# UCSC-nanopore-cgl/margin

Hardware: AMD Instinct MI355X
Metric: het-sites x reads phased/sec (30x ONT synthetic chunks, end to end: every merge level + final sweep) (higher is better)
Workload: dtype int32

## Files before the change

margin_amd/csrc/mrp_kernels.hip:

```cpp
#include <hip/hip_runtime.h>
#include <stdint.h>

#include "mrp_device.h"
#include "mrp_internal.h"
#include "mrp_kernels.h"
#include "mrp_wave.h"
#include "../../include/margin_rphmm.h"

static __device__ __forceinline__ double i32_to_log(int32_t v) {
    return v == MRP_NEG_I32 ? -__builtin_inf() : (double) v;
}
static __device__ __forceinline__ int32_t add_i32(int32_t a, int32_t b) {
    return a == MRP_NEG_I32 ? MRP_NEG_I32 : a + b;
}

__global__ void __launch_bounds__(256) mrp_planes_kernel(const PlaneCol *__restrict__ pcols_all,
                                                         const int32_t *__restrict__ list, int64_t n_cols,
                                                         const int64_t *__restrict__ read_byte_off,
                                                         uint64_t *__restrict__ planes,
                                                         uint32_t *__restrict__ slot_total,
                                                         uint32_t *__restrict__ slot_bytes, int filter) {
    const int lane = threadIdx.x & (WAVE - 1);
    const int wave = __builtin_amdgcn_readfirstlane((int) (threadIdx.x / WAVE));
    const int64_t wave_stride = (int64_t) gridDim.x * (blockDim.x / WAVE);
    int64_t col = (int64_t) blockIdx.x * (blockDim.x / WAVE) + wave;
    if (col >= n_cols) return;
#define PLANE_COL(i) (pcols_all + (list ? (int64_t) __builtin_amdgcn_readfirstlane(list[i]) : (i)))
    PlaneCol c = k_load(PLANE_COL(col));
    int64_t my_off = lane < c.depth ? read_byte_off[c.read_off + lane] : 0;
    for (; col < n_cols; col += wave_stride) {
    const int64_t ncol = col + wave_stride < n_cols ? col + wave_stride : col;
    const PlaneCol cn = k_load(PLANE_COL(ncol));
    const int64_t next_off = lane < cn.depth ? read_byte_off[cn.read_off + lane] : 0;
    const bool active = lane < c.depth;
    const uint8_t *__restrict__ src = c.pool + my_off;
#define PLANE_U 8
    const int n_slots_here = (filter && !c.need_planes) ? 0 : c.n_slots;
    for (int s0 = 0; s0 < n_slots_here; s0 += PLANE_U) {
        uint32_t bytes[PLANE_U];
#pragma unroll
        for (int u = 0; u < PLANE_U; u++) bytes[u] = (active && s0 + u < c.n_slots) ? src[s0 + u] : 0u;
#pragma unroll
        for (int u = 0; u < PLANE_U; u++) {
            const int s = s0 + u;
            if (s < c.n_slots) {
                const uint32_t byte = bytes[u];
                uint32_t packed = byte << (8 * (lane & 3));
                packed |= __shfl_xor(packed, 1, WAVE);
                packed |= __shfl_xor(packed, 2, WAVE);
                if ((lane & 3) == 0) slot_bytes[(c.slot_off + s) * 16 + (lane >> 2)] = packed;
                uint32_t total = __builtin_amdgcn_udot4(packed, 0x01010101u, 0u, false);
                total += __shfl_xor(total, 4, WAVE);
                total += __shfl_xor(total, 8, WAVE);
                total += __shfl_xor(total, 16, WAVE);
                total += __shfl_xor(total, 32, WAVE);
                if (lane == 0) slot_total[c.slot_off + s] = total;
                if (c.need_planes) {
                    uint64_t mine = 0;
#pragma unroll
                    for (int b = 0; b < MRP_ALLELE_LOG_PROB_BITS; b++) {
                        const uint64_t v = __ballot((byte >> b) & 1u);
                        if (lane == b) mine = v;
                    }
                    if (lane < MRP_ALLELE_LOG_PROB_BITS) planes[(c.slot_off + s) * MRP_ALLELE_LOG_PROB_BITS + lane] = mine;
                }
            }
        }
    }
    c = cn;
    my_off = next_off;
    }
#undef PLANE_U
#undef PLANE_COL
}

struct __attribute__((packed, aligned(1))) pack_u32 { uint32_t v; };
__global__ void __launch_bounds__(256) mrp_pack_kernel(const PlaneCol *__restrict__ pcols, const int32_t *__restrict__ list,
                                                       int64_t n_list, const int64_t *__restrict__ read_byte_off,
                                                       uint32_t *__restrict__ slot_total, uint32_t *__restrict__ slot_bytes, int filter) {
    const int64_t q = ((int64_t) blockIdx.x * blockDim.x + threadIdx.x) >> 4;
    const int w = threadIdx.x & 15;
    if (q >= n_list) return;
    const PlaneCol c = pcols[list ? list[q] : q];
    if (filter && c.need_planes) return;
    int64_t off[4];
#pragma unroll
    for (int r = 0; r < 4; r++) {
        const int read = 4 * w + r;
        off[r] = read < c.depth ? read_byte_off[c.read_off + read] : -1;
    }
    for (int s = 0; s < c.n_slots; s += 4) {
        uint32_t v[4];
#pragma unroll
        for (int r = 0; r < 4; r++)
            v[r] = off[r] >= 0 ? ((const __attribute__((address_space(1))) pack_u32 *) (c.pool + off[r] + s))->v : 0u;
        const uint32_t ta = __builtin_amdgcn_perm(v[1], v[0], 0x05010400u), tb = __builtin_amdgcn_perm(v[1], v[0], 0x07030602u);
        const uint32_t tc = __builtin_amdgcn_perm(v[3], v[2], 0x05010400u), td = __builtin_amdgcn_perm(v[3], v[2], 0x07030602u);
        const uint32_t o[4] = {__builtin_amdgcn_perm(tc, ta, 0x05040100u), __builtin_amdgcn_perm(tc, ta, 0x07060302u),
                               __builtin_amdgcn_perm(td, tb, 0x05040100u), __builtin_amdgcn_perm(td, tb, 0x07060302u)};
        const int left = c.n_slots - s;
#pragma unroll
        for (int j = 0; j < 4; j++)
            if (j < left) slot_bytes[(c.slot_off + s + j) * 16 + w] = o[j];
        uint32_t t01 = __builtin_amdgcn_udot4(o[0], 0x01010101u, 0u, false) | (__builtin_amdgcn_udot4(o[1], 0x01010101u, 0u, false) << 16);
        uint32_t t23 = __builtin_amdgcn_udot4(o[2], 0x01010101u, 0u, false) | (__builtin_amdgcn_udot4(o[3], 0x01010101u, 0u, false) << 16);
        t01 += (uint32_t) __builtin_amdgcn_update_dpp(0, (int) t01, 0x128, 0xf, 0xf, false); t23 += (uint32_t) __builtin_amdgcn_update_dpp(0, (int) t23, 0x128, 0xf, 0xf, false);
        t01 += (uint32_t) __builtin_amdgcn_update_dpp(0, (int) t01, 0x124, 0xf, 0xf, false); t23 += (uint32_t) __builtin_amdgcn_update_dpp(0, (int) t23, 0x124, 0xf, 0xf, false);
        t01 += (uint32_t) __builtin_amdgcn_update_dpp(0, (int) t01, 0x122, 0xf, 0xf, false); t23 += (uint32_t) __builtin_amdgcn_update_dpp(0, (int) t23, 0x122, 0xf, 0xf, false);
        t01 += (uint32_t) __builtin_amdgcn_update_dpp(0, (int) t01, 0x121, 0xf, 0xf, false); t23 += (uint32_t) __builtin_amdgcn_update_dpp(0, (int) t23, 0x121, 0xf, 0xf, false);
        if (w < 4 && w < left) slot_total[c.slot_off + s + w] = w == 0 ? (t01 & 0xFFFFu) : (w == 1 ? (t01 >> 16) : (w == 2 ? (t23 & 0xFFFFu) : (t23 >> 16)));
    }
}

hipError_t mrp_launch_planes(const MrpBatchDev &d, hipStream_t stream) {
    if (d.n_cols == 0) return hipSuccess;
    const int waves = 4;
    const bool split = d.pack_list != nullptr || d.plane_list != nullptr || d.list_filter != 0;
    const int64_t n_planes = split ? d.n_plane_list : d.n_cols;
    if (n_planes > 0) {
        int64_t grid = (n_planes + waves - 1) / waves;
        if (grid > MRP_PERSISTENT_GRID) grid = MRP_PERSISTENT_GRID;
        hipLaunchKernelGGL(mrp_planes_kernel, dim3((unsigned) grid), dim3(waves * WAVE), 0, stream, d.pcols,
                           split ? d.plane_list : (const int32_t *) nullptr, n_planes, d.read_byte_off, d.planes, d.slot_total,
                           d.slot_bytes, d.list_filter);
    }
    if (split && d.n_pack_list > 0) {
        const int64_t grid = (d.n_pack_list * 16 + 255) / 256;
        hipLaunchKernelGGL(mrp_pack_kernel, dim3((unsigned) grid), dim3(256), 0, stream, d.pcols, d.pack_list, d.n_pack_list,
                           d.read_byte_off, d.slot_total, d.slot_bytes, d.list_filter);
    }
    return hipGetLastError();
}

template <bool NARROW>
static __device__ __forceinline__ uint32_t allele_cost(const uint64_t (&w)[8], uint64_t P) {
    uint32_t r = 0;
    const uint32_t plo = (uint32_t) P, phi = (uint32_t) (P >> 32);
#pragma unroll
    for (int b = 0; b < 8; b++) {
        uint32_t c = (uint32_t) __popc((uint32_t) w[b] & plo);
        if (!NARROW) c += (uint32_t) __popc((uint32_t) (w[b] >> 32) & phi);
        r += c << b;
    }
    return r;
}

template <int CPT, bool NARROW>
static __device__ __forceinline__ void column_cost_plain(const DevCol &c, K_AS(uint32_t) allele_number,
                                                         K_AS(uint64_t) planes, K_AS(uint32_t) slot_total,
                                                         const uint64_t (&P)[CPT], uint32_t (&cost)[CPT]) {
    int64_t slot = c.slot_off;
#pragma unroll
    for (int j = 0; j < CPT; j++) cost[j] = 0;
    for (int s = 0; s < c.n_sites; s++) {
        const uint32_t A = allele_number[c.site_start + s];
        uint32_t m1[CPT], m2[CPT];
#pragma unroll
        for (int j = 0; j < CPT; j++) { m1[j] = 0xFFFFFFFFu; m2[j] = 0xFFFFFFFFu; }
        for (uint32_t a = 0; a < A; a++) {
            K_AS(uint64_t) pl = planes + (slot + a) * 8;
            uint64_t w[8];
#pragma unroll
            for (int b = 0; b < 8; b++) w[b] = pl[b];
            const uint32_t t = slot_total[slot + a];
#pragma unroll
            for (int j = 0; j < CPT; j++) {
                const uint32_t lp = allele_cost<NARROW>(w, P[j]);
                m1[j] = min(m1[j], lp);
                m2[j] = min(m2[j], t - lp);
            }
        }
#pragma unroll
        for (int j = 0; j < CPT; j++) cost[j] += m1[j] + m2[j];
        slot += A;
    }
}

static __device__ uint32_t column_cost_ancestor(const DevCol &c, const DevChunk &ch, K_AS(uint64_t) planes,
                                                K_AS(uint32_t) slot_total, uint64_t P) {
    int64_t slot = c.slot_off;
    uint32_t cost = 0;
    for (int s = 0; s < c.n_sites; s++) {
        const int site = c.site_start + s;
        const uint32_t A = K_PTR(uint32_t, ch.allele_number)[site];
        K_AS(uint16_t) sub = K_PTR(uint16_t, ch.sub) + K_PTR(uint32_t, ch.sub_offset)[site];
        K_AS(uint16_t) prior = K_PTR(uint16_t, ch.prior) + K_PTR(uint32_t, ch.allele_offset)[site];
        uint32_t h1[MRP_MAX_ALLELES], h2[MRP_MAX_ALLELES];
        for (uint32_t a = 0; a < A; a++) {
            K_AS(uint64_t) pl = planes + (slot + a) * 8;
            uint64_t w[8];
#pragma unroll
            for (int b = 0; b < 8; b++) w[b] = pl[b];
            const uint32_t lp = allele_cost<false>(w, P);
            h1[a] = lp;
            h2[a] = slot_total[slot + a] - lp;
        }
        uint32_t g = 0xFFFFFFFFu;
        for (uint32_t i = 0; i < A; i++) {
            uint32_t a1 = 0xFFFFFFFFu, a2 = 0xFFFFFFFFu;
            for (uint32_t k = 0; k < A; k++) {
                const uint32_t sc = sub[i * A + k];
                a1 = min(a1, h1[k] + sc);
                a2 = min(a2, h2[k] + sc);
            }
            g = min(g, a1 + a2 + (uint32_t) prior[i]);
        }
        cost += g;
        slot += A;
    }
    return cost;
}

template <int NW>
static __device__ __forceinline__ void expand_partition(uint64_t P, uint32_t (&sel)[NW]) {
    const uint32_t lo = (uint32_t) P, hi = (uint32_t) (P >> 32);
#pragma unroll
    for (int w = 0; w < NW; w++) {
        const uint32_t nib = w < 8 ? ((lo >> (4 * w)) & 0xFu) : ((hi >> (4 * (w - 8))) & 0xFu);
        sel[w] = (nib * 0x00204081u) & 0x01010101u;
    }
}

template <int CP, int NW>
static __device__ __forceinline__ void column_cost_dot(int64_t slot0, int n_slots, int A, K_AS(uint32_t) slot_bytes,
                                                       K_AS(uint32_t) slot_total, const uint64_t (&P)[CP],
                                                       uint32_t (&cost)[CP]) {
    uint32_t sel[CP][NW];
    uint32_t m1[CP], m2[CP];
#pragma unroll
    for (int j = 0; j < CP; j++) {
        expand_partition<NW>(P[j], sel[j]);
        cost[j] = 0;
        m1[j] = 0xFFFFFFFFu;
        m2[j] = 0xFFFFFFFFu;
    }
    uint32_t B0[NW], B1[NW];
    uint32_t tot0, tot1 = 0;
    {
        K_AS(uint32_t) p = slot_bytes + slot0 * 16;
#pragma unroll
        for (int w = 0; w < NW; w++) B0[w] = p[w];
        tot0 = slot_total[slot0];
    }
    int a = 0;
#define DOT_STEP(BC, TC, BN, TN, g)                                                            \
    {                                                                                            \
        const int gn_ = (g) + 1 < n_slots ? (g) + 1 : (g);                                       \
        K_AS(uint32_t) p_ = slot_bytes + (slot0 + gn_) * 16;                                     \
        _Pragma("unroll") for (int w = 0; w < NW; w++) BN[w] = p_[w];                            \
        TN = slot_total[slot0 + gn_];                                                            \
        uint32_t lp_[CP];                                                                        \
        _Pragma("unroll") for (int j = 0; j < CP; j++) lp_[j] = 0;                               \
                                   \
        _Pragma("unroll") for (int w = 0; w < NW; w++) {                                         \
            _Pragma("unroll") for (int j = 0; j < CP; j++)                                       \
                lp_[j] = __builtin_amdgcn_udot4(BC[w], sel[j][w], lp_[j], false);                \
        }                                                                                        \
        _Pragma("unroll") for (int j = 0; j < CP; j++) {                                         \
            m1[j] = min(m1[j], lp_[j]);                                                          \
            m2[j] = min(m2[j], TC - lp_[j]);                                                     \
        }                                                                                        \
        if (++a == A) {                                                       \
            a = 0;                                                                               \
            _Pragma("unroll") for (int j = 0; j < CP; j++) {                                     \
                cost[j] += m1[j] + m2[j];                                                        \
                m1[j] = 0xFFFFFFFFu;                                                             \
                m2[j] = 0xFFFFFFFFu;                                                             \
            }                                                                                    \
        }                                                                                        \
    }
    for (int g = 0; g < n_slots; g += 2) {
        DOT_STEP(B0, tot0, B1, tot1, g)
        if (g + 1 < n_slots) DOT_STEP(B1, tot1, B0, tot0, g + 1)
    }
#undef DOT_STEP
}

template <int NW, int EMIT_CP>
static __device__ __forceinline__ void emit_tile(const MrpBatchDev &d, const EmitTile &t, int lane, int pair0) {
    K_AS(uint32_t) slot_bytes = K_PTR(uint32_t, d.slot_bytes);
    K_AS(uint32_t) slot_total = K_PTR(uint32_t, d.slot_total);
    const uint64_t mask = t.depth < 64 ? ~(0xFFFFFFFFFFFFFFFFull << t.depth) : 0xFFFFFFFFFFFFFFFFull;
    const int n_slots = t.n_sites * t.uniform_alleles;
    uint64_t Pe[EMIT_CP], Po[EMIT_CP];
    bool has_odd[EMIT_CP], paired[EMIT_CP];
    bool any_unpaired = false;
#pragma unroll
    for (int u = 0; u < EMIT_CP; u++) {
        const int e = 2 * (pair0 + u * WAVE + lane);
        Pe[u] = e < t.n ? d.partition[t.cell_off + e] : 0ull;
        has_odd[u] = e + 1 < t.n;
        Po[u] = has_odd[u] ? d.partition[t.cell_off + e + 1] : 0ull;
        paired[u] = has_odd[u] && Po[u] == (~Pe[u] & mask);
        any_unpaired |= has_odd[u] && !paired[u];
    }
    uint32_t cost[EMIT_CP];
    column_cost_dot<EMIT_CP, NW>(t.slot_off, n_slots, t.uniform_alleles, slot_bytes, slot_total, Pe, cost);
#pragma unroll
    for (int u = 0; u < EMIT_CP; u++) {
        const int e = 2 * (pair0 + u * WAVE + lane);
        if (e < t.n) d.cell_cost[t.cell_off + e] = cost[u];
        if (paired[u]) d.cell_cost[t.cell_off + e + 1] = cost[u];
    }
    if (__any(any_unpaired)) {
        column_cost_dot<EMIT_CP, NW>(t.slot_off, n_slots, t.uniform_alleles, slot_bytes, slot_total, Po, cost);
#pragma unroll
        for (int u = 0; u < EMIT_CP; u++) {
            const int e = 2 * (pair0 + u * WAVE + lane);
            if (has_odd[u] && !paired[u]) d.cell_cost[t.cell_off + e + 1] = cost[u];
        }
    }
}

__global__ void __launch_bounds__(256) mrp_emission_kernel(MrpBatchDev d, const EmitTile *__restrict__ tiles,
                                                           int64_t n_tiles) {
    const int lane = threadIdx.x & (WAVE - 1);
    const int wave = __builtin_amdgcn_readfirstlane((int) (threadIdx.x / WAVE));
    const int64_t tile = (int64_t) blockIdx.x * (blockDim.x / WAVE) + wave;
    if (tile >= n_tiles) return;
    const EmitTile t = k_load(tiles + tile);
    if (t.depth <= 16) emit_tile<4, 4>(d, t, lane, 0);
    else if (t.depth <= 32) emit_tile<8, 4>(d, t, lane, 0);
    else if (t.depth <= 48) {
        emit_tile<12, 2>(d, t, lane, 0);
        if (t.n > 256) emit_tile<12, 2>(d, t, lane, 128);
    } else {
        emit_tile<16, 2>(d, t, lane, 0);
        if (t.n > 256) emit_tile<16, 2>(d, t, lane, 128);
    }
}

__global__ void __launch_bounds__(256) mrp_emission_general_kernel(MrpBatchDev d, const EmitTile *__restrict__ tiles,
                                                                   int64_t n_tiles) {
    const int lane = threadIdx.x & (WAVE - 1);
    const int wave = __builtin_amdgcn_readfirstlane((int) (threadIdx.x / WAVE));
    const int64_t tile = (int64_t) blockIdx.x * (blockDim.x / WAVE) + wave;
    if (tile >= n_tiles) return;
    const EmitTile t = k_load(tiles + tile);
    const DevCol c = k_load(d.cols + t.col);
    const DevChunk ch = k_load(d.chunks + c.chunk);
    K_AS(uint64_t) planes = K_PTR(uint64_t, d.planes);
    K_AS(uint32_t) slot_total = K_PTR(uint32_t, d.slot_total);
    const bool ancestor = (t.flags & MRP_FLAG_INCLUDE_ANCESTOR_SUB_PROB) != 0;
    for (int idx = lane; idx < t.n; idx += WAVE) {
        const uint64_t P[1] = {d.partition[t.cell_off + idx]};
        uint32_t cost[1];
        if (ancestor) cost[0] = column_cost_ancestor(c, ch, planes, slot_total, P[0]);
        else column_cost_plain<1, false>(c, K_PTR(uint32_t, ch.allele_number), planes, slot_total, P, cost);
        d.cell_cost[t.cell_off + idx] = cost[0];
    }
}

__global__ void __launch_bounds__(256) mrp_tiles_kernel(const DevCol *__restrict__ cols, const TileCol *__restrict__ tc, int64_t n_cols,
                                                        EmitTile *__restrict__ tiles) {
    const int64_t col = (int64_t) blockIdx.x * blockDim.x + threadIdx.x;
    if (col >= n_cols) return;
    const DevCol c = cols[col];
    const TileCol t0 = tc[col];
    int64_t at = t0.first;
    for (int32_t off = 0; off < c.n_cells; off += MRP_EMIT_TILE, at++) {
        EmitTile t;
        t.cell_off = c.cell_off + off;
        t.slot_off = c.slot_off;
        t.n = c.n_cells - off < MRP_EMIT_TILE ? c.n_cells - off : MRP_EMIT_TILE;
        t.col = (int32_t) col;
        t.n_sites = c.n_sites;
        t.uniform_alleles = t0.uniform_alleles;
        t.depth = c.depth;
        t.flags = c.flags;
        t.pad[0] = 0;
        t.pad[1] = 0;
        tiles[at] = t;
    }
}

hipError_t mrp_launch_tiles(const DevCol *cols_dev, const TileCol *tilecols_dev, int64_t n_cols, EmitTile *tiles_dev, hipStream_t stream) {
    if (n_cols <= 0) return hipSuccess;
    hipLaunchKernelGGL(mrp_tiles_kernel, dim3((unsigned) ((n_cols + 255) / 256)), dim3(256), 0, stream, cols_dev, tilecols_dev, n_cols, tiles_dev);
    return hipGetLastError();
}

hipError_t mrp_launch_emission(const MrpBatchDev &d, const EmitTile *tiles_dev, int64_t n_fast, int64_t n_general,
                               hipStream_t stream) {
    const int waves = 4;
    if (n_fast > 0)
        hipLaunchKernelGGL(mrp_emission_kernel, dim3((unsigned) ((n_fast + waves - 1) / waves)), dim3(waves * WAVE), 0,
                           stream, d, tiles_dev, n_fast);
    if (n_general > 0)
        hipLaunchKernelGGL(mrp_emission_general_kernel, dim3((unsigned) ((n_general + waves - 1) / waves)),
                           dim3(waves * WAVE), 0, stream, d, tiles_dev + n_fast, n_general);
    return hipGetLastError();
}

#define SWEEP_R 8
#define SWEEP_WIN 128

struct SweepShared {
    int32_t *cur;
    int32_t *nxt;
    int32_t *red;
    int2 *dsc;
    int win0;
};

static __device__ __forceinline__ void stage_window(SweepShared &S, const SweepCol *cols, int K, int win0, int tid, int T) {
    __syncthreads();
    for (int i = tid; i < SWEEP_WIN; i += T) {
        const int k = win0 + i;
        if (k >= 0 && k < K) S.dsc[i] = make_int2(cols[k].n_cells, cols[k].n_merge);
    }
    S.win0 = win0;
    __syncthreads();
}
static __device__ __forceinline__ int2 col_desc(const SweepShared &S, int k) {
    const int2 v = S.dsc[k - S.win0];
    return make_int2(__builtin_amdgcn_readfirstlane(v.x), __builtin_amdgcn_readfirstlane(v.y));
}

__global__ void __launch_bounds__(1024)
mrp_sweep_i32_kernel(MrpBatchDev d, const int32_t *__restrict__ order, int max_merge) {
    extern __shared__ __attribute__((aligned(16))) int32_t lds[];
    SweepShared S;
    S.cur = lds;
    S.nxt = lds + max_merge;
    S.red = lds + 2 * max_merge;
    S.dsc = reinterpret_cast<int2 *>(lds + 2 * max_merge + 4);
    S.win0 = 0;

    const int tid = threadIdx.x, T = blockDim.x, lane = threadIdx.x & (WAVE - 1);
    const bool backward = (blockIdx.x & 1) != 0;
    const int64_t hmm_index = K_PTR(int32_t, order)[blockIdx.x >> 1];
    const DevHmm h = k_load(d.hmms + hmm_index);
    const SweepCol *cols = d.scols + h.col0;
    const int K = h.n_cols;
    const SweepCol first_col = k_load(cols);
    const int N = (int) h.n_cells;
    const int G = (N + 3) / 4;
    const int Q = (G + T - 1) / T;
    const uint32_t *__restrict__ cost = d.cell_cost + first_col.cell_off;
    const uint32_t *__restrict__ np = d.cell_np + first_col.cell_off;
    int32_t *__restrict__ out_f = d.cell_f32 + first_col.cell_off;
    int32_t *__restrict__ out_b = d.cell_b32 + first_col.cell_off;
    int32_t *__restrict__ out_mf = d.merge_f32 + first_col.mcell_off;
    int32_t *__restrict__ out_mb = d.merge_b32 + first_col.mcell_off;

    typedef uint32_t u32x4 __attribute__((ext_vector_type(4)));
    typedef int32_t i32x4 __attribute__((ext_vector_type(4)));
    u32x4 rc0, rc1, rc2, rc3, rc4, rc5, rc6, rc7, rn0, rn1, rn2, rn3, rn4, rn5, rn6, rn7;
#define RING_LOAD(i, q)                                                                              \
    {                                                                                                \
        int g_ = (q) * T + tid;                                                                      \
        g_ = g_ < 0 ? 0 : (g_ > G - 1 ? G - 1 : g_);                                                 \
        asm volatile("global_load_dwordx4 %0, %2, off\n\tglobal_load_dwordx4 %1, %3, off"            \
                     : "=&v"(rc##i), "=&v"(rn##i)                                                    \
                     : "v"(cost + 4 * g_), "v"(np + 4 * g_)                                          \
                     : "memory");                                                                    \
    }
#ifdef MRP_SAFE_WAIT
#define RING_WAIT(i, n) asm volatile("s_waitcnt vmcnt(0)" : "+v"(rc##i), "+v"(rn##i)::"memory");
#else
#define RING_WAIT(i, n) asm volatile("s_waitcnt vmcnt(" #n ")" : "+v"(rc##i), "+v"(rn##i)::"memory");
#endif
    if (!backward) {
        RING_LOAD(0, 0) RING_LOAD(1, 1) RING_LOAD(2, 2) RING_LOAD(3, 3)
        RING_LOAD(4, 4) RING_LOAD(5, 5) RING_LOAD(6, 6) RING_LOAD(7, 7)
    } else {
        RING_LOAD(0, Q - 1) RING_LOAD(1, Q - 2) RING_LOAD(2, Q - 3) RING_LOAD(3, Q - 4)
        RING_LOAD(4, Q - 5) RING_LOAD(5, Q - 6) RING_LOAD(6, Q - 7) RING_LOAD(7, Q - 8)
    }

    for (int i = tid; i < 2 * max_merge; i += T) lds[i] = MRP_NEG_I32;
    if (tid < 4) S.red[tid] = MRP_NEG_I32;
    stage_window(S, cols, K, 0, tid, T);

#define STORE4(out, p0, ok, v)                                                                               \
    {                                                                                                        \
        int32_t *dst_ = (ok) ? (out) + (p0) : scratch;                                                       \
        const i32x4 q_ = {v[0], v[1], v[2], v[3]};                                                           \
        *reinterpret_cast<i32x4 *>(dst_) = q_;                                                               \
    }
    int32_t *scratch = d.cell_f32 + d.n_cells;

#define RING_DRAIN() asm volatile("s_waitcnt vmcnt(0)"                                                                          \
                 : "+v"(rc0), "+v"(rc1), "+v"(rc2), "+v"(rc3), "+v"(rc4), "+v"(rc5), "+v"(rc6), "+v"(rc7),       \
                   "+v"(rn0), "+v"(rn1), "+v"(rn2), "+v"(rn3), "+v"(rn4), "+v"(rn5), "+v"(rn6), "+v"(rn7)        \
                 :                                                                                             \
                 : "memory");

    if (!backward) {
        int k = 0;
        int2 dk = col_desc(S, 0);
        int cs = 0, ce = dk.x;
        int mo = 0;
        int32_t local_max = MRP_NEG_I32;
#define FWD_ROUND(i, qq, nw)                                                                               \
    RING_WAIT(i, nw)                                                                                         \
    {                                                                                                        \
    const int pos0 = 4 * ((qq) * T + tid);                                                                   \
    int32_t fv[4] = {MRP_NEG_I32, MRP_NEG_I32, MRP_NEG_I32, MRP_NEG_I32};                                    \
    if ((qq) < Q && k < K) {                                                                                 \
        const int rend = 4 * ((qq) + 1) * T;                                                                 \
        for (;;) {                                                                                           \
            const bool first = (k == 0), last = (k == K - 1);                                                \
                        \
            bool act[4];                                                                                     \
            bool any_act = false;                                                                            \
            _Pragma("unroll") for (int j = 0; j < 4; j++) {                                                  \
                const int p = pos0 + j;                                                                      \
                act[j] = (p >= cs) & (p < ce);                                                               \
                any_act |= act[j];                                                                           \
            }                                                                                                \
            if (__any(any_act)) {                                                                            \
                int32_t fp[4] = {0, 0, 0, 0};                                                                \
                if (!first) {                                                                                \
                    _Pragma("unroll") for (int j = 0; j < 4; j++)                                            \
                        fp[j] = S.cur[act[j] ? (rn##i[j] >> 16) : lane];           \
                }                                                                                            \
                _Pragma("unroll") for (int j = 0; j < 4; j++) {                                              \
                    const int32_t v = add_i32(fp[j], -(int32_t) rc##i[j]);                                   \
                    fv[j] = act[j] ? v : fv[j];                                                              \
                    const int32_t val = act[j] ? v : MRP_NEG_I32;                                            \
                    if (!last) atomicMax(&S.nxt[act[j] ? (rn##i[j] & 0xFFFFu) : lane], val);       \
                    else local_max = max(local_max, val);                                                    \
                }                                                                                            \
            }                                                                                                \
            if (ce > rend) break;                                \
                                                                                   \
            if (last) {                                                                                      \
                local_max = wave_max_i32(local_max);                                                         \
                if ((tid & (WAVE - 1)) == 0) atomicMax(&S.red[0], local_max);                                \
                k = K;                                                                                       \
                break;                                                                                       \
            }                                                                                                \
            if (k + 1 >= S.win0 + SWEEP_WIN) stage_window(S, cols, K, k, tid, T);                            \
            const int2 dn = col_desc(S, k + 1);                                                              \
            lds_barrier();                                                                                   \
            for (int m = tid; m < dk.y; m += T) out_mf[mo + m] = S.nxt[m];                       \
            if (k + 2 < K) for (int m = tid; m < dn.y; m += T) S.cur[m] = MRP_NEG_I32;                       \
            lds_barrier();                                                                                   \
            { int32_t *t_ = S.cur; S.cur = S.nxt; S.nxt = t_; }                                              \
            mo += dk.y;                                                                                      \
            k++;                                                                                             \
            dk = dn;                                                                                         \
            cs = ce;                                                                                         \
            ce = cs + dk.x;                                                                                  \
            if (cs >= rend) break;                                                                           \
        }                                                                                                    \
    }                                                                                                        \
    STORE4(out_f, pos0, (qq) < Q && pos0 < N, fv)                                                            \
    }                                                                                                        \
    RING_LOAD(i, (qq) + SWEEP_R)
        FWD_ROUND(0, 0, 14) FWD_ROUND(1, 1, 15) FWD_ROUND(2, 2, 16) FWD_ROUND(3, 3, 17)
        FWD_ROUND(4, 4, 18) FWD_ROUND(5, 5, 19) FWD_ROUND(6, 6, 20) FWD_ROUND(7, 7, 21)
        for (int q0 = SWEEP_R; q0 < Q; q0 += SWEEP_R) {
            FWD_ROUND(0, q0, 21) FWD_ROUND(1, q0 + 1, 21) FWD_ROUND(2, q0 + 2, 21) FWD_ROUND(3, q0 + 3, 21)
            FWD_ROUND(4, q0 + 4, 21) FWD_ROUND(5, q0 + 5, 21) FWD_ROUND(6, q0 + 6, 21) FWD_ROUND(7, q0 + 7, 21)
        }
#undef FWD_ROUND
        RING_DRAIN()
        __syncthreads();
        const double total = i32_to_log(S.red[0]);
        for (int kk = tid; kk < K; kk += T) d.col_total[h.col0 + kk] = total;
        if (tid == 0) d.hmm_fb[2 * hmm_index] = total;
    }
    else {
        int k = K - 1;
        if (k < S.win0 || k >= S.win0 + SWEEP_WIN) stage_window(S, cols, K, max(0, K - SWEEP_WIN), tid, T);
        int2 dk = col_desc(S, k);
        int ce = N, cs = N - dk.x;
        int mo = (int) h.n_merge;
        if (K >= 2) {
            if (k - 1 < S.win0) stage_window(S, cols, K, max(0, k - SWEEP_WIN + 1), tid, T);
            const int2 dp = col_desc(S, k - 1);
            for (int m = tid; m < dp.y; m += T) S.nxt[m] = MRP_NEG_I32;
        }
        lds_barrier();
        int32_t local_max = MRP_NEG_I32;
#define BWD_ROUND(i, qq, nw)                                                                                 \
    RING_WAIT(i, nw)                                                                                         \
    {                                                                                                        \
    const int pos0 = 4 * ((qq) * T + tid);                                                                   \
    int32_t bv[4] = {MRP_NEG_I32, MRP_NEG_I32, MRP_NEG_I32, MRP_NEG_I32};                                    \
    if ((qq) >= 0 && k >= 0) {                                                                               \
        const int rbeg = 4 * (qq) * T;                                                                       \
        for (;;) {                                                                                           \
            const bool first = (k == 0), last = (k == K - 1);                                                \
            bool act[4];                                                                                     \
            bool any_act = false;                                                                            \
            _Pragma("unroll") for (int j = 0; j < 4; j++) {                                                  \
                const int p = pos0 + j;                                                                      \
                act[j] = (p >= cs) & (p < ce);                                                               \
                any_act |= act[j];                                                                           \
            }                                                                                                \
            if (__any(any_act)) {                                                                            \
                int32_t bn[4] = {0, 0, 0, 0};                                                                \
                if (!last) {                                                                                 \
                    _Pragma("unroll") for (int j = 0; j < 4; j++)                                            \
                        bn[j] = S.cur[act[j] ? (rn##i[j] & 0xFFFFu) : lane];       \
                }                                                                                            \
                _Pragma("unroll") for (int j = 0; j < 4; j++) {                                              \
                    bv[j] = act[j] ? bn[j] : bv[j];                                                          \
                    const int32_t pv = act[j] ? add_i32(bn[j], -(int32_t) rc##i[j]) : MRP_NEG_I32;           \
                    if (!first) atomicMax(&S.nxt[act[j] ? (rn##i[j] >> 16) : lane], pv);                     \
                    else local_max = max(local_max, pv);                                                     \
                }                                                                                            \
            }                                                                                                \
            if (cs < rbeg) break;                            \
            if (first) {                                                                                     \
                local_max = wave_max_i32(local_max);                                                         \
                if ((tid & (WAVE - 1)) == 0) atomicMax(&S.red[1], local_max);                                \
                k = -1;                                                                                      \
                break;                                                                                       \
            }                                                                                                \
            if (k - 2 >= 0 && k - 2 < S.win0) stage_window(S, cols, K, max(0, k - SWEEP_WIN + 1), tid, T);   \
            else if (k - 1 < S.win0) stage_window(S, cols, K, max(0, k - SWEEP_WIN + 1), tid, T);            \
            const int2 dp = col_desc(S, k - 1);                                                              \
            const int n_clear = (k >= 2) ? col_desc(S, k - 2).y : 0;                                         \
            lds_barrier();                                                                                   \
            for (int m = tid; m < dp.y; m += T) out_mb[mo - dp.y + m] = S.nxt[m];                \
            for (int m = tid; m < n_clear; m += T) S.cur[m] = MRP_NEG_I32;                                   \
            lds_barrier();                                                                                   \
            { int32_t *t_ = S.cur; S.cur = S.nxt; S.nxt = t_; }                                              \
            mo -= dp.y;                                                                                      \
            k--;                                                                                             \
            dk = dp;                                                                                         \
            ce = cs;                                                                                         \
            cs = ce - dk.x;                                                                                  \
            if (ce <= rbeg) break;                                                                           \
        }                                                                                                    \
    }                                                                                                        \
    STORE4(out_b, pos0, (qq) >= 0 && pos0 < N, bv)                                                           \
    }                                                                                                        \
    RING_LOAD(i, (qq) - SWEEP_R)
        BWD_ROUND(0, Q - 1, 14) BWD_ROUND(1, Q - 2, 15) BWD_ROUND(2, Q - 3, 16) BWD_ROUND(3, Q - 4, 17)
        BWD_ROUND(4, Q - 5, 18) BWD_ROUND(5, Q - 6, 19) BWD_ROUND(6, Q - 7, 20) BWD_ROUND(7, Q - 8, 21)
        for (int q0 = Q - 1 - SWEEP_R; q0 >= 0; q0 -= SWEEP_R) {
            BWD_ROUND(0, q0, 21) BWD_ROUND(1, q0 - 1, 21) BWD_ROUND(2, q0 - 2, 21) BWD_ROUND(3, q0 - 3, 21)
            BWD_ROUND(4, q0 - 4, 21) BWD_ROUND(5, q0 - 5, 21) BWD_ROUND(6, q0 - 6, 21) BWD_ROUND(7, q0 - 7, 21)
        }
#undef BWD_ROUND
        RING_DRAIN()
        __syncthreads();
        if (tid == 0) d.hmm_fb[2 * hmm_index + 1] = i32_to_log(S.red[1]);
    }
#undef RING_DRAIN
#undef RING_LOAD
#undef RING_WAIT
#undef STORE4
}

hipError_t mrp_launch_sweep_i32(const MrpBatchDev &d, const int32_t *order_dev, int64_t n, int block_threads,
                                int max_merge, hipStream_t stream) {
    if (n == 0) return hipSuccess;
    if (max_merge < WAVE) max_merge = WAVE;
    const size_t lds = (size_t) (2 * max_merge + 4) * sizeof(int32_t) + SWEEP_WIN * sizeof(int2);
    auto k = mrp_sweep_i32_kernel;
    static PerDeviceOnce once;
    const hipError_t attr_status = once.run([] {
        return hipFuncSetAttribute((const void *) mrp_sweep_i32_kernel, hipFuncAttributeMaxDynamicSharedMemorySize, 160 * 1024);
    });
    if (attr_status != hipSuccess) return attr_status;
    hipLaunchKernelGGL(k, dim3((unsigned) (2 * n)), dim3(block_threads), lds, stream, d, order_dev, max_merge);
    return hipGetLastError();
}

static __device__ __forceinline__ double log_add_exact(double x, double y) {
    if (x == -__builtin_inf()) return y;
    if (y == -__builtin_inf()) return x;
    return x > y ? x + log(1.0 + exp(y - x)) : y + log(1.0 + exp(x - y));
}
static __device__ __forceinline__ double log_add_p(double a, double b, bool max_not_sum) {
    return max_not_sum ? (a > b ? a : b) : log_add_exact(a, b);
}
static __device__ __forceinline__ double load_agent(double *p) {
    return __hip_atomic_load(p, __ATOMIC_RELAXED, __HIP_MEMORY_SCOPE_AGENT);
}
static __device__ void atomic_log_add_p(double *addr, double v, bool max_not_sum) {
    if (v == -__builtin_inf()) return;
    unsigned long long *a = (unsigned long long *) addr;
    unsigned long long old = __hip_atomic_load(a, __ATOMIC_RELAXED, __HIP_MEMORY_SCOPE_AGENT);
    while (true) {
        const double cur = __longlong_as_double((long long) old);
        const double nv = log_add_p(cur, v, max_not_sum);
        const unsigned long long nvb = (unsigned long long) __double_as_longlong(nv);
        if (nvb == old) return;
        const unsigned long long seen = atomicCAS(a, old, nvb);
        if (seen == old) return;
        old = seen;
    }
}
static __device__ __forceinline__ double wave_log_add_p(double v, bool max_not_sum) {
#pragma unroll
    for (int o = 32; o > 0; o >>= 1) {
        const double t = __shfl_xor(v, o, WAVE);
        v = log_add_p(v, t, max_not_sum);
    }
    return v;
}

__global__ void __launch_bounds__(1024) mrp_sweep_f64_kernel(MrpBatchDev d, const int32_t *__restrict__ order) {
    const int tid = threadIdx.x, T = blockDim.x;
    const int64_t hmm_index = K_PTR(int32_t, order)[blockIdx.x];
    const DevHmm h = k_load(d.hmms + hmm_index);
    const SweepCol *cols = d.scols + h.col0;
    const int K = h.n_cols;
    const bool wide = h.wide_idx != 0;
    const bool max_not_sum = (h.flags & MRP_FLAG_MAX_NOT_SUM) != 0;
    const double NEG = -__builtin_inf();
    double *hmm_f = d.hmm_fb + 2 * hmm_index, *hmm_b = hmm_f + 1;

    for (int k = 0; k < K; k++) {
        const SweepCol c = k_load(cols + k);
        const bool first = (k == 0), last = (k == K - 1);
        const SweepCol pc = k_load(cols + (first ? k : k - 1));
        double local = NEG;
        for (int idx = tid; idx < c.n_cells; idx += T) {
            const int64_t g = c.cell_off + idx;
            const double e = -((double) d.cell_cost[g]);
            const uint32_t nx = wide ? d.cell_next[g] : (d.cell_np[g] & 0xFFFFu);
            const uint32_t pv = wide ? d.cell_prev[g] : (d.cell_np[g] >> 16);
            double fv = first ? 0.0 : load_agent(&d.merge_f[pc.mcell_off + pv]);
            fv += e;
            d.cell_f[g] = fv;
            if (!last) atomic_log_add_p(&d.merge_f[c.mcell_off + nx], fv, max_not_sum);
            else local = log_add_p(local, fv, max_not_sum);
        }
        if (last) {
            local = wave_log_add_p(local, max_not_sum);
            if ((tid & (WAVE - 1)) == 0) atomic_log_add_p(hmm_f, local, max_not_sum);
        }
        __syncthreads();
    }
    for (int k = K - 1; k >= 0; k--) {
        const SweepCol c = k_load(cols + k);
        const bool first = (k == 0), last = (k == K - 1);
        const SweepCol pc = k_load(cols + (first ? k : k - 1));
        double local_b = NEG, local_t = NEG;
        for (int idx = tid; idx < c.n_cells; idx += T) {
            const int64_t g = c.cell_off + idx;
            const uint32_t nx = wide ? d.cell_next[g] : (d.cell_np[g] & 0xFFFFu);
            const uint32_t pv = wide ? d.cell_prev[g] : (d.cell_np[g] >> 16);
            double p = -((double) d.cell_cost[g]);
            double bv = 0.0;
            if (!last) { bv = load_agent(&d.merge_b[c.mcell_off + nx]); p += bv; }
            d.cell_b[g] = bv;
            if (!first) atomic_log_add_p(&d.merge_b[pc.mcell_off + pv], p, max_not_sum);
            else local_b = log_add_p(local_b, p, max_not_sum);
            local_t = log_add_p(local_t, d.cell_f[g] + bv, max_not_sum);
        }
        if (first) {
            local_b = wave_log_add_p(local_b, max_not_sum);
            if ((tid & (WAVE - 1)) == 0) atomic_log_add_p(hmm_b, local_b, max_not_sum);
        }
        local_t = wave_log_add_p(local_t, max_not_sum);
        if ((tid & (WAVE - 1)) == 0) atomic_log_add_p(&d.col_total[h.col0 + k], local_t, max_not_sum);
        __syncthreads();
    }
}

hipError_t mrp_launch_sweep_f64(const MrpBatchDev &d, const int32_t *order_dev, int64_t n, int block_threads,
                                hipStream_t stream) {
    if (n == 0) return hipSuccess;
    hipLaunchKernelGGL(mrp_sweep_f64_kernel, dim3((unsigned) n), dim3(block_threads), 0, stream, d, order_dev);
    return hipGetLastError();
}

#define LSE_KEY_NEG_INF ((int32_t) 0x807FFFFF)
static __device__ __forceinline__ int32_t lse_key_up(double v) {
    float f = (float) v;
    if ((double) f < v) f = __int_as_float(__float_as_int(f) + (f >= 0.0f ? 1 : -1));
    const int32_t b = __float_as_int(f);
    return b >= 0 ? b : (int32_t) (b ^ 0x7FFFFFFF);
}
static __device__ __forceinline__ double lse_key_value(int32_t k) {
    return (double) __int_as_float(k >= 0 ? k : (int32_t) (k ^ 0x7FFFFFFF));
}
#define LSE_FIX 1125899906842624.0
struct LseAcc { double m, s; };
static __device__ __forceinline__ void lse_push(LseAcc &a, double v) {
    if (v == -__builtin_inf()) return;
    if (v > a.m) { a.s = a.s * exp(a.m - v) + 1.0; a.m = v; }
    else a.s += exp(v - a.m);
}
static __device__ __forceinline__ void lse_merge(LseAcc &a, double m, double s) {
    if (m == -__builtin_inf()) return;
    if (m > a.m) { a.s = a.s * exp(a.m - m) + s; a.m = m; }
    else a.s += s * exp(m - a.m);
}
static __device__ __forceinline__ double lse_value(const LseAcc &a) { return a.m == -__builtin_inf() ? a.m : a.m + log(a.s); }

template <bool CUR_LDS>
__global__ void __launch_bounds__(512) mrp_sweep_lse_kernel(MrpBatchDev d, const int32_t *__restrict__ order, int max_merge) {
    extern __shared__ __attribute__((aligned(16))) unsigned char lse_lds[];
    unsigned long long *acc = reinterpret_cast<unsigned long long *>(lse_lds);
    double *cur = reinterpret_cast<double *>(lse_lds + 8 * (size_t) max_merge);
    double *part = cur + (CUR_LDS ? max_merge : 0);
    int32_t *rkey = reinterpret_cast<int32_t *>(part + 16);
    const int tid = threadIdx.x, T = blockDim.x, lane = tid & (WAVE - 1), wave = tid / WAVE, n_waves = T / WAVE;
    const int64_t hmm_index = K_PTR(int32_t, order)[blockIdx.x];
    const DevHmm h = k_load(d.hmms + hmm_index);
    const SweepCol *cols = d.scols + h.col0;
    const int K = h.n_cols;
    const double NEG = -__builtin_inf();
    for (int m = tid; m < max_merge; m += T) { rkey[m] = LSE_KEY_NEG_INF; acc[m] = 0ull; if (CUR_LDS) cur[m] = NEG; }
    __syncthreads();

    auto finish = [&](int m) -> double {
        const unsigned long long a = acc[m];
        const double v = a ? lse_key_value(rkey[m]) + log((double) a * (1.0 / LSE_FIX)) : NEG;
        rkey[m] = LSE_KEY_NEG_INF;
        acc[m] = 0ull;
        return v;
    };

    for (int k = 0; k < K; k++) {
        const SweepCol c = k_load(cols + k);
        const bool first = (k == 0), last = (k == K - 1);
        const double *prev_mf = d.merge_f + k_load(cols + (first ? k : k - 1)).mcell_off;
        for (int idx = tid; idx < c.n_cells; idx += T) {
            const int64_t g = c.cell_off + idx;
            const uint32_t np = d.cell_np[g];
            const double fv = (first ? 0.0 : (CUR_LDS ? cur[np >> 16] : load_agent(const_cast<double *>(prev_mf + (np >> 16))))) - (double) d.cell_cost[g];
            d.cell_f[g] = fv;
            if (fv != NEG) atomicMax(&rkey[last ? 0u : (np & 0xFFFFu)], lse_key_up(fv));
        }
        __syncthreads();
        for (int idx = tid; idx < c.n_cells; idx += T) {
            const int64_t g = c.cell_off + idx;
            const uint32_t to = last ? 0u : (d.cell_np[g] & 0xFFFFu);
            const double fv = d.cell_f[g];
            if (fv != NEG) atomicAdd(&acc[to], (unsigned long long) (exp(fv - lse_key_value(rkey[to])) * LSE_FIX));
        }
        __syncthreads();
        if (!last) {
            for (int m = tid; m < c.n_merge; m += T) {
                const double v = finish(m);
                if (CUR_LDS) cur[m] = v;
                d.merge_f[c.mcell_off + m] = v;
            }
        } else if (tid == 0) d.hmm_fb[2 * hmm_index] = finish(0);
        __syncthreads();
    }
    for (int k = K - 1; k >= 0; k--) {
        const SweepCol c = k_load(cols + k);
        const bool first = (k == 0), last = (k == K - 1);
        const SweepCol pc = k_load(cols + (first ? k : k - 1));
        LseAcc tot = {NEG, 0.0};
        for (int idx = tid; idx < c.n_cells; idx += T) {
            const int64_t g = c.cell_off + idx;
            const uint32_t np = d.cell_np[g];
            const double bv = last ? 0.0 : (CUR_LDS ? cur[np & 0xFFFFu] : load_agent(d.merge_b + c.mcell_off + (np & 0xFFFFu)));
            d.cell_b[g] = bv;
            const double p = bv - (double) d.cell_cost[g];
            if (p != NEG) atomicMax(&rkey[first ? 0u : (np >> 16)], lse_key_up(p));
            lse_push(tot, d.cell_f[g] + bv);
        }
#pragma unroll
        for (int o = 32; o > 0; o >>= 1) {
            const double om = __shfl_xor(tot.m, o, WAVE), os = __shfl_xor(tot.s, o, WAVE);
            LseAcc lo = (lane & o) ? LseAcc{om, os} : tot, hi = (lane & o) ? tot : LseAcc{om, os};
            lse_merge(lo, hi.m, hi.s);
            tot = lo;
        }
        if (lane == 0) { part[2 * wave] = tot.m; part[2 * wave + 1] = tot.s; }
        __syncthreads();
        for (int idx = tid; idx < c.n_cells; idx += T) {
            const int64_t g = c.cell_off + idx;
            const uint32_t to = first ? 0u : (d.cell_np[g] >> 16);
            const double p = d.cell_b[g] - (double) d.cell_cost[g];
            if (p != NEG) atomicAdd(&acc[to], (unsigned long long) (exp(p - lse_key_value(rkey[to])) * LSE_FIX));
        }
        if (tid == 0) {
            LseAcc t = {NEG, 0.0};
            for (int w = 0; w < n_waves; w++) lse_merge(t, part[2 * w], part[2 * w + 1]);
            d.col_total[h.col0 + k] = lse_value(t);
        }
        __syncthreads();
        if (!first) {
            for (int m = tid; m < pc.n_merge; m += T) {
                const double v = finish(m);
                if (CUR_LDS) cur[m] = v;
                d.merge_b[pc.mcell_off + m] = v;
            }
        } else if (tid == 0) d.hmm_fb[2 * hmm_index + 1] = finish(0);
        __syncthreads();
    }
}

hipError_t mrp_launch_sweep_lse(const MrpBatchDev &d, const int32_t *order_dev, int64_t n, int max_merge, hipStream_t stream) {
    if (n == 0) return hipSuccess;
    if (max_merge < 1) max_merge = 1;
    max_merge = (max_merge + 1) & ~1;
    const bool cur_lds = max_merge <= MRP_LSE_CUR_LDS_MAX_MERGE;
    const size_t lds = (size_t) max_merge * (cur_lds ? 20 : 12) + 16 * sizeof(double);
    static PerDeviceOnce once;
    const hipError_t attr_status = once.run([] {
        hipError_t e = hipFuncSetAttribute((const void *) mrp_sweep_lse_kernel<true>, hipFuncAttributeMaxDynamicSharedMemorySize, 160 * 1024);
        if (e == hipSuccess) e = hipFuncSetAttribute((const void *) mrp_sweep_lse_kernel<false>, hipFuncAttributeMaxDynamicSharedMemorySize, 160 * 1024);
        return e;
    });
    if (attr_status != hipSuccess) return attr_status;
    if (cur_lds) hipLaunchKernelGGL(mrp_sweep_lse_kernel<true>, dim3((unsigned) n), dim3(512), lds, stream, d, order_dev, max_merge);
    else hipLaunchKernelGGL(mrp_sweep_lse_kernel<false>, dim3((unsigned) n), dim3(512), lds, stream, d, order_dev, max_merge);
    return hipGetLastError();
}

__global__ void mrp_fill_f64_kernel(double *p, int64_t n, double v) {
    for (int64_t i = (int64_t) blockIdx.x * blockDim.x + threadIdx.x; i < n; i += (int64_t) gridDim.x * blockDim.x)
        p[i] = v;
}
hipError_t mrp_launch_fill_f64(double *p, int64_t n, double v, hipStream_t stream) {
    if (n <= 0) return hipSuccess;
    int64_t grid = (n + 255) / 256;
    if (grid > 2048) grid = 2048;
    hipLaunchKernelGGL(mrp_fill_f64_kernel, dim3((unsigned) grid), dim3(256), 0, stream, p, n, v);
    return hipGetLastError();
}

__global__ void mrp_emissions_kernel(const DevCol *__restrict__ col, const DevChunk *__restrict__ chunks,
                                     const uint64_t *__restrict__ planes, const uint32_t *__restrict__ slot_total,
                                     uint32_t flags, int64_t n_cells, const uint64_t *__restrict__ partitions,
                                     double *__restrict__ out) {
    const DevCol c = k_load(col);
    const DevChunk ch = k_load(chunks + c.chunk);
    const int64_t i = (int64_t) blockIdx.x * blockDim.x + threadIdx.x;
    if (i >= n_cells) return;
    const uint64_t P[1] = {partitions[i]};
    uint32_t cost[1];
    if (flags & MRP_FLAG_INCLUDE_ANCESTOR_SUB_PROB)
        cost[0] = column_cost_ancestor(c, ch, K_PTR(uint64_t, planes), K_PTR(uint32_t, slot_total), P[0]);
    else
        column_cost_plain<1, false>(c, K_PTR(uint32_t, ch.allele_number), K_PTR(uint64_t, planes),
                                    K_PTR(uint32_t, slot_total), P, cost);
    out[i] = -((double) cost[0]);
}
hipError_t mrp_launch_emissions(const DevCol *col_dev, const DevChunk *chunks, const uint64_t *planes,
                                const uint32_t *slot_total, uint32_t flags, int64_t n_cells,
                                const uint64_t *partitions, double *out, hipStream_t stream) {
    if (n_cells <= 0) return hipSuccess;
    hipLaunchKernelGGL(mrp_emissions_kernel, dim3((unsigned) ((n_cells + 255) / 256)), dim3(256), 0, stream, col_dev,
                       chunks, planes, slot_total, flags, n_cells, partitions, out);
    return hipGetLastError();
}
```

Baseline: 445.9 million.

## Shrink sweep load ring to four, add per-wave column skipping and register descriptors

Cuts the sweep kernel's prefetch ring from eight to four register sets and drops the launch bound to 512 threads, freeing VGPRs so more waves can be resident. Column descriptors are now held in two registers per lane and fetched with readlane instead of an LDS read. Each wave decides from its own cell range whether to skip a column, take an unmasked fast path, or take the masked path. Merge-column copy and clear loops are restructured to batch four loads. The shallower ring exposes more memory latency, and block sizes above 512 are now rejected.

```diff
diff --git a/margin_amd/csrc/mrp_kernels.hip b/margin_amd/csrc/mrp_kernels.hip
--- a/margin_amd/csrc/mrp_kernels.hip
+++ b/margin_amd/csrc/mrp_kernels.hip
@@ -392,14 +392,25 @@
     return hipGetLastError();
 }
 
-#define SWEEP_R 8
+#ifndef MRP_SWEEP_RING
+#define MRP_SWEEP_RING 4
+#endif
+#define SWEEP_R MRP_SWEEP_RING
+static_assert(SWEEP_R == 4 || SWEEP_R == 8, "the ring is written out for four or eight register sets");
 #define SWEEP_WIN 128
+#define SWEEP_MAX_T 512
+#define SWEEP_LAUNCH_BOUND (SWEEP_R == 4 ? SWEEP_MAX_T : 1024)
+static_assert(SWEEP_WIN == 2 * WAVE, "a wave keeps the window's descriptors in two registers per field");
+
+typedef uint32_t u32x4 __attribute__((ext_vector_type(4)));
+typedef int32_t i32x4 __attribute__((ext_vector_type(4)));
 
 struct SweepShared {
     int32_t *cur;
     int32_t *nxt;
     int32_t *red;
     int2 *dsc;
+    int2 dlo, dhi;
     int win0;
 };
 
@@ -411,13 +422,67 @@
     }
     S.win0 = win0;
     __syncthreads();
+    S.dlo = S.dsc[tid & (WAVE - 1)];
+    S.dhi = S.dsc[WAVE + (tid & (WAVE - 1))];
 }
 static __device__ __forceinline__ int2 col_desc(const SweepShared &S, int k) {
-    const int2 v = S.dsc[k - S.win0];
-    return make_int2(__builtin_amdgcn_readfirstlane(v.x), __builtin_amdgcn_readfirstlane(v.y));
-}
-
-__global__ void __launch_bounds__(1024)
+    const int i = __builtin_amdgcn_readfirstlane(k - S.win0);
+    if (i < WAVE) return make_int2(__builtin_amdgcn_readlane(S.dlo.x, i), __builtin_amdgcn_readlane(S.dlo.y, i));
+    return make_int2(__builtin_amdgcn_readlane(S.dhi.x, i - WAVE), __builtin_amdgcn_readlane(S.dhi.y, i - WAVE));
+}
+
+template <bool MASKED, bool FWD>
+static __device__ __forceinline__ void sweep_cells(const int32_t *cur, int32_t *nxt, const u32x4 rc, const u32x4 rn, int pos0, int cs,
+                                                   int ce, bool gather, bool scatter, int lane, int32_t (&keep)[4], int32_t &local_max) {
+    bool act[4] = {true, true, true, true};
+    if (MASKED) {
+#pragma unroll
+        for (int j = 0; j < 4; j++) act[j] = (pos0 + j >= cs) & (pos0 + j < ce);
+    }
+    int32_t g[4] = {0, 0, 0, 0}, val[4];
+    if (gather) {
+#pragma unroll
+        for (int j = 0; j < 4; j++) {
+            const int from = (int) (FWD ? rn[j] >> 16 : rn[j] & 0xFFFFu);
+            g[j] = cur[MASKED && !act[j] ? lane : from];
+        }
+    }
+#pragma unroll
+    for (int j = 0; j < 4; j++) {
+        const int32_t s = add_i32(g[j], -(int32_t) rc[j]);
+        const int32_t kept = FWD ? s : g[j];
+        keep[j] = MASKED && !act[j] ? keep[j] : kept;
+        val[j] = MASKED && !act[j] ? MRP_NEG_I32 : s;
+    }
+    if (scatter) {
+#pragma unroll
+        for (int j = 0; j < 4; j++) {
+            const int to = (int) (FWD ? rn[j] & 0xFFFFu : rn[j] >> 16);
+            atomicMax(&nxt[MASKED && !act[j] ? lane : to], val[j]);
+        }
+    } else {
+#pragma unroll
+        for (int j = 0; j < 4; j++) local_max = max(local_max, val[j]);
+    }
+}
+
+static __device__ __forceinline__ void merge_column_out(int32_t *__restrict__ out, const int32_t *col, int n, int tid, int T) {
+#pragma clang loop vectorize(disable) unroll(disable)
+    for (int m0 = 0; m0 < n; m0 += 4 * T) {
+        int32_t v[4];
+#pragma unroll
+        for (int j = 0; j < 4; j++) v[j] = col[min(m0 + j * T + tid, n - 1)];
+#pragma unroll
+        for (int j = 0; j < 4; j++)
+            if (m0 + j * T + tid < n) out[m0 + j * T + tid] = v[j];
+    }
+}
+static __device__ __forceinline__ void merge_column_clear(int32_t *col, int n, int tid, int T) {
+#pragma clang loop vectorize(disable) unroll(disable)
+    for (int m = tid; m < n; m += T) col[m] = MRP_NEG_I32;
+}
+
+__global__ void __launch_bounds__(SWEEP_LAUNCH_BOUND)
 mrp_sweep_i32_kernel(MrpBatchDev d, const int32_t *__restrict__ order, int max_merge) {
     extern __shared__ __attribute__((aligned(16))) int32_t lds[];
     SweepShared S;
@@ -428,6 +493,7 @@
     S.win0 = 0;
 
     const int tid = threadIdx.x, T = blockDim.x, lane = threadIdx.x & (WAVE - 1);
+    const int wave0 = __builtin_amdgcn_readfirstlane(tid & ~(WAVE - 1));
     const bool backward = (blockIdx.x & 1) != 0;
     const int64_t hmm_index = K_PTR(int32_t, order)[blockIdx.x >> 1];
     const DevHmm h = k_load(d.hmms + hmm_index);
@@ -444,9 +510,15 @@
     int32_t *__restrict__ out_mf = d.merge_f32 + first_col.mcell_off;
     int32_t *__restrict__ out_mb = d.merge_b32 + first_col.mcell_off;
 
-    typedef uint32_t u32x4 __attribute__((ext_vector_type(4)));
-    typedef int32_t i32x4 __attribute__((ext_vector_type(4)));
+#if SWEEP_R == 8
     u32x4 rc0, rc1, rc2, rc3, rc4, rc5, rc6, rc7, rn0, rn1, rn2, rn3, rn4, rn5, rn6, rn7;
+#define RING_EACH(X) X(0) X(1) X(2) X(3) X(4) X(5) X(6) X(7)
+#else
+    u32x4 rc0, rc1, rc2, rc3, rn0, rn1, rn2, rn3;
+#define RING_EACH(X) X(0) X(1) X(2) X(3)
+#endif
+#define RING_WAIT_STEADY (3 * (SWEEP_R - 1))
+#define RING_WAIT_FIRST_LAP(i) (2 * (SWEEP_R - 1) + (i))
 #define RING_LOAD(i, q)                                                                              \
     {                                                                                                \
         int g_ = (q) * T + tid;                                                                      \
@@ -459,19 +531,17 @@
 #ifdef MRP_SAFE_WAIT
 #define RING_WAIT(i, n) asm volatile("s_waitcnt vmcnt(0)" : "+v"(rc##i), "+v"(rn##i)::"memory");
 #else
-#define RING_WAIT(i, n) asm volatile("s_waitcnt vmcnt(" #n ")" : "+v"(rc##i), "+v"(rn##i)::"memory");
+#define RING_WAIT(i, n) asm volatile("s_waitcnt vmcnt(%2)" : "+v"(rc##i), "+v"(rn##i) : "i"(n) : "memory");
 #endif
-    if (!backward) {
-        RING_LOAD(0, 0) RING_LOAD(1, 1) RING_LOAD(2, 2) RING_LOAD(3, 3)
-        RING_LOAD(4, 4) RING_LOAD(5, 5) RING_LOAD(6, 6) RING_LOAD(7, 7)
-    } else {
-        RING_LOAD(0, Q - 1) RING_LOAD(1, Q - 2) RING_LOAD(2, Q - 3) RING_LOAD(3, Q - 4)
-        RING_LOAD(4, Q - 5) RING_LOAD(5, Q - 6) RING_LOAD(6, Q - 7) RING_LOAD(7, Q - 8)
-    }
+#define PROLOGUE_LOAD(i) RING_LOAD(i, backward ? Q - 1 - (i) : (i))
+    RING_EACH(PROLOGUE_LOAD)
+#undef PROLOGUE_LOAD
 
     for (int i = tid; i < 2 * max_merge; i += T) lds[i] = MRP_NEG_I32;
     if (tid < 4) S.red[tid] = MRP_NEG_I32;
     stage_window(S, cols, K, 0, tid, T);
+    asm volatile("s_waitcnt vmcnt(0)" ::: "memory");
+    __builtin_amdgcn_sched_barrier(0);
 
 #define STORE4(out, p0, ok, v)                                                                               \
     {                                                                                                        \
@@ -481,11 +551,18 @@
     }
     int32_t *scratch = d.cell_f32 + d.n_cells;
 
+#if SWEEP_R == 8
 #define RING_DRAIN() asm volatile("s_waitcnt vmcnt(0)"                                                                          \
                  : "+v"(rc0), "+v"(rc1), "+v"(rc2), "+v"(rc3), "+v"(rc4), "+v"(rc5), "+v"(rc6), "+v"(rc7),       \
                    "+v"(rn0), "+v"(rn1), "+v"(rn2), "+v"(rn3), "+v"(rn4), "+v"(rn5), "+v"(rn6), "+v"(rn7)        \
                  :                                                                                             \
                  : "memory");
+#else
+#define RING_DRAIN() asm volatile("s_waitcnt vmcnt(0)"                                                                          \
+                 : "+v"(rc0), "+v"(rc1), "+v"(rc2), "+v"(rc3), "+v"(rn0), "+v"(rn1), "+v"(rn2), "+v"(rn3)        \
+                 :                                                                                             \
+                 : "memory");
+#endif
 
     if (!backward) {
         int k = 0;
@@ -500,29 +577,15 @@
     int32_t fv[4] = {MRP_NEG_I32, MRP_NEG_I32, MRP_NEG_I32, MRP_NEG_I32};                                    \
     if ((qq) < Q && k < K) {                                                                                 \
         const int rend = 4 * ((qq) + 1) * T;                                                                 \
+        const int wbeg = 4 * ((qq) * T + wave0), wend = wbeg + 4 * WAVE;   \
         for (;;) {                                                                                           \
             const bool first = (k == 0), last = (k == K - 1);                                                \
-                        \
-            bool act[4];                                                                                     \
-            bool any_act = false;                                                                            \
-            _Pragma("unroll") for (int j = 0; j < 4; j++) {                                                  \
-                const int p = pos0 + j;                                                                      \
-                act[j] = (p >= cs) & (p < ce);                                                               \
-                any_act |= act[j];                                                                           \
-            }                                                                                                \
-            if (__any(any_act)) {                                                                            \
-                int32_t fp[4] = {0, 0, 0, 0};                                                                \
-                if (!first) {                                                                                \
-                    _Pragma("unroll") for (int j = 0; j < 4; j++)                                            \
-                        fp[j] = S.cur[act[j] ? (rn##i[j] >> 16) : lane];           \
-                }                                                                                            \
-                _Pragma("unroll") for (int j = 0; j < 4; j++) {                                              \
-                    const int32_t v = add_i32(fp[j], -(int32_t) rc##i[j]);                                   \
-                    fv[j] = act[j] ? v : fv[j];                                                              \
-                    const int32_t val = act[j] ? v : MRP_NEG_I32;                                            \
-                    if (!last) atomicMax(&S.nxt[act[j] ? (rn##i[j] & 0xFFFFu) : lane], val);       \
-                    else local_max = max(local_max, val);                                                    \
-                }                                                                                            \
+                                                       \
+            if (ce > wbeg && cs < wend) {                                                                    \
+                if (cs <= wbeg && ce >= wend)                                                                \
+                    sweep_cells<false, true>(S.cur, S.nxt, rc##i, rn##i, pos0, cs, ce, !first, !last, lane, fv, local_max); \
+                else                                                                                         \
+                    sweep_cells<true, true>(S.cur, S.nxt, rc##i, rn##i, pos0, cs, ce, !first, !last, lane, fv, local_max); \
             }                                                                                                \
             if (ce > rend) break;                                \
                                                                                    \
@@ -535,8 +598,8 @@
             if (k + 1 >= S.win0 + SWEEP_WIN) stage_window(S, cols, K, k, tid, T);                            \
             const int2 dn = col_desc(S, k + 1);                                                              \
             lds_barrier();                                                                                   \
-            for (int m = tid; m < dk.y; m += T) out_mf[mo + m] = S.nxt[m];                       \
-            if (k + 2 < K) for (int m = tid; m < dn.y; m += T) S.cur[m] = MRP_NEG_I32;                       \
+            merge_column_out(out_mf + mo, S.nxt, dk.y, tid, T);                                              \
+            if (k + 2 < K) merge_column_clear(S.cur, dn.y, tid, T);                                          \
             lds_barrier();                                                                                   \
             { int32_t *t_ = S.cur; S.cur = S.nxt; S.nxt = t_; }                                              \
             mo += dk.y;                                                                                      \
@@ -550,11 +613,13 @@
     STORE4(out_f, pos0, (qq) < Q && pos0 < N, fv)                                                            \
     }                                                                                                        \
     RING_LOAD(i, (qq) + SWEEP_R)
-        FWD_ROUND(0, 0, 14) FWD_ROUND(1, 1, 15) FWD_ROUND(2, 2, 16) FWD_ROUND(3, 3, 17)
-        FWD_ROUND(4, 4, 18) FWD_ROUND(5, 5, 19) FWD_ROUND(6, 6, 20) FWD_ROUND(7, 7, 21)
+#define FIRST_LAP(i) FWD_ROUND(i, i, RING_WAIT_FIRST_LAP(i))
+        RING_EACH(FIRST_LAP)
+#undef FIRST_LAP
         for (int q0 = SWEEP_R; q0 < Q; q0 += SWEEP_R) {
-            FWD_ROUND(0, q0, 21) FWD_ROUND(1, q0 + 1, 21) FWD_ROUND(2, q0 + 2, 21) FWD_ROUND(3, q0 + 3, 21)
-            FWD_ROUND(4, q0 + 4, 21) FWD_ROUND(5, q0 + 5, 21) FWD_ROUND(6, q0 + 6, 21) FWD_ROUND(7, q0 + 7, 21)
+#define STEADY(i) FWD_ROUND(i, q0 + (i), RING_WAIT_STEADY)
+            RING_EACH(STEADY)
+#undef STEADY
         }
 #undef FWD_ROUND
         RING_DRAIN()
@@ -583,27 +648,14 @@
     int32_t bv[4] = {MRP_NEG_I32, MRP_NEG_I32, MRP_NEG_I32, MRP_NEG_I32};                                    \
     if ((qq) >= 0 && k >= 0) {                                                                               \
         const int rbeg = 4 * (qq) * T;                                                                       \
+        const int wbeg = 4 * ((qq) * T + wave0), wend = wbeg + 4 * WAVE;   \
         for (;;) {                                                                                           \
             const bool first = (k == 0), last = (k == K - 1);                                                \
-            bool act[4];                                                                                     \
-            bool any_act = false;                                                                            \
-            _Pragma("unroll") for (int j = 0; j < 4; j++) {                                                  \
-                const int p = pos0 + j;                                                                      \
-                act[j] = (p >= cs) & (p < ce);                                                               \
-                any_act |= act[j];                                                                           \
-            }                                                                                                \
-            if (__any(any_act)) {                                                                            \
-                int32_t bn[4] = {0, 0, 0, 0};                                                                \
-                if (!last) {                                                                                 \
-                    _Pragma("unroll") for (int j = 0; j < 4; j++)                                            \
-                        bn[j] = S.cur[act[j] ? (rn##i[j] & 0xFFFFu) : lane];       \
-                }                                                                                            \
-                _Pragma("unroll") for (int j = 0; j < 4; j++) {                                              \
-                    bv[j] = act[j] ? bn[j] : bv[j];                                                          \
-                    const int32_t pv = act[j] ? add_i32(bn[j], -(int32_t) rc##i[j]) : MRP_NEG_I32;           \
-                    if (!first) atomicMax(&S.nxt[act[j] ? (rn##i[j] >> 16) : lane], pv);                     \
-                    else local_max = max(local_max, pv);                                                     \
-                }                                                                                            \
+            if (ce > wbeg && cs < wend) {                                   \
+                if (cs <= wbeg && ce >= wend)                                                                \
+                    sweep_cells<false, false>(S.cur, S.nxt, rc##i, rn##i, pos0, cs, ce, !last, !first, lane, bv, local_max); \
+                else                                                                                         \
+                    sweep_cells<true, false>(S.cur, S.nxt, rc##i, rn##i, pos0, cs, ce, !last, !first, lane, bv, local_max); \
             }                                                                                                \
             if (cs < rbeg) break;                            \
             if (first) {                                                                                     \
@@ -612,13 +664,13 @@
                 k = -1;                                                                                      \
                 break;                                                                                       \
             }                                                                                                \
-            if (k - 2 >= 0 && k - 2 < S.win0) stage_window(S, cols, K, max(0, k - SWEEP_WIN + 1), tid, T);   \
-            else if (k - 1 < S.win0) stage_window(S, cols, K, max(0, k - SWEEP_WIN + 1), tid, T);            \
+            if ((k - 2 >= 0 && k - 2 < S.win0) || k - 1 < S.win0)                                            \
+                stage_window(S, cols, K, max(0, k - SWEEP_WIN + 1), tid, T);                                 \
             const int2 dp = col_desc(S, k - 1);                                                              \
             const int n_clear = (k >= 2) ? col_desc(S, k - 2).y : 0;                                         \
             lds_barrier();                                                                                   \
-            for (int m = tid; m < dp.y; m += T) out_mb[mo - dp.y + m] = S.nxt[m];                \
-            for (int m = tid; m < n_clear; m += T) S.cur[m] = MRP_NEG_I32;                                   \
+            merge_column_out(out_mb + (mo - dp.y), S.nxt, dp.y, tid, T);                                     \
+            merge_column_clear(S.cur, n_clear, tid, T);                                                      \
             lds_barrier();                                                                                   \
             { int32_t *t_ = S.cur; S.cur = S.nxt; S.nxt = t_; }                                              \
             mo -= dp.y;                                                                                      \
@@ -632,11 +684,13 @@
     STORE4(out_b, pos0, (qq) >= 0 && pos0 < N, bv)                                                           \
     }                                                                                                        \
     RING_LOAD(i, (qq) - SWEEP_R)
-        BWD_ROUND(0, Q - 1, 14) BWD_ROUND(1, Q - 2, 15) BWD_ROUND(2, Q - 3, 16) BWD_ROUND(3, Q - 4, 17)
-        BWD_ROUND(4, Q - 5, 18) BWD_ROUND(5, Q - 6, 19) BWD_ROUND(6, Q - 7, 20) BWD_ROUND(7, Q - 8, 21)
+#define FIRST_LAP(i) BWD_ROUND(i, Q - 1 - (i), RING_WAIT_FIRST_LAP(i))
+        RING_EACH(FIRST_LAP)
+#undef FIRST_LAP
         for (int q0 = Q - 1 - SWEEP_R; q0 >= 0; q0 -= SWEEP_R) {
-            BWD_ROUND(0, q0, 21) BWD_ROUND(1, q0 - 1, 21) BWD_ROUND(2, q0 - 2, 21) BWD_ROUND(3, q0 - 3, 21)
-            BWD_ROUND(4, q0 - 4, 21) BWD_ROUND(5, q0 - 5, 21) BWD_ROUND(6, q0 - 6, 21) BWD_ROUND(7, q0 - 7, 21)
+#define STEADY(i) BWD_ROUND(i, q0 - (i), RING_WAIT_STEADY)
+            RING_EACH(STEADY)
+#undef STEADY
         }
 #undef BWD_ROUND
         RING_DRAIN()
@@ -646,12 +700,16 @@
 #undef RING_DRAIN
 #undef RING_LOAD
 #undef RING_WAIT
+#undef RING_WAIT_STEADY
+#undef RING_WAIT_FIRST_LAP
+#undef RING_EACH
 #undef STORE4
 }
 
 hipError_t mrp_launch_sweep_i32(const MrpBatchDev &d, const int32_t *order_dev, int64_t n, int block_threads,
                                 int max_merge, hipStream_t stream) {
     if (n == 0) return hipSuccess;
+    if (block_threads < WAVE || block_threads > SWEEP_MAX_T || block_threads % WAVE) return hipErrorInvalidValue;
     if (max_merge < WAVE) max_merge = WAVE;
     const size_t lds = (size_t) (2 * max_merge + 4) * sizeof(int32_t) + SWEEP_WIN * sizeof(int2);
     auto k = mrp_sweep_i32_kernel;
```

New measurement: 419.8 million. -5.9%, worse.
